# openhumanoids/pronto

Hardware: AMD Instinct MI355X
Metric: EKF predict+update steps/sec (batched filters), 15-state, 1000 Hz IMU (higher is better)
Workload: dtype f64

## Files before the change

pronto_amd/csrc/rbis_coop.hpp:

```cpp
#pragma once

#include "rbis_device.hpp"

namespace pb {

template <int NS>
struct Coop {
  static constexpr bool HB = (NS == 21);
  static constexpr int NSC = HB ? 15 : 9;
  static constexpr int NPC = NSC * (NSC + 1) / 2;
  static constexpr int NB_ = HB ? 6 : 0;
  static constexpr bool LL_IN_P = !HB;
  static constexpr int XCH_LLI = 9 + 3 * NSC;
  static constexpr int NXCH = 9 + 3 * NSC + (LL_IN_P ? 1 : 0);
  PB_HD static constexpr int fullc(int s) { return core_full(s); }
  PB_HD static constexpr int fullp(int p) { return passive_full(p); }
};

struct ProcBlocks {
  double a_mw[3];
  double a_g[3];
  double a_mv[3];
  double A_R[9];
  double A_RV[9];
// ... 73 lines not shown
using CorrGpfYawPos = Corr<false, 5, 6, 7, 8>;
using CorrGpfChiPos = Corr<false, 3, 4, 5, 6, 7, 8>;
using CorrGpfZ = Corr<false, 8>;
struct CorrInputs {
  double z[6], rd[6], qm[4];
  double ro[15] = { 0, 0, 0, 0, 0, 0, 0, 0, 0, 0, 0, 0, 0, 0, 0 };
  bool upd;
};
template <int NS, class CORR>
struct CoopX {
  using C = Coop<NS>;
  static constexpr int M = CORR::M;
  static constexpr int X2_L = C::NXCH, X2_ID = X2_L + M * (M - 1) / 2, X2_YD = X2_ID + M, X2_W = X2_YD + M,
                       X2_LLI = X2_W + C::NSC * M;
  static constexpr int NXCH = (M == 0) ? C::NXCH : X2_LLI + (C::LL_IN_P ? 1 : 0);
  static constexpr int XCH_LEG = C::NXCH, XCH_FOOT = XCH_LEG + 10, NXCH_LEG = (NXCH > XCH_FOOT + 14) ? NXCH : XCH_FOOT + 14;
  static constexpr int X6_ID = 0, X6_YD = 3, X6_LLI = 6, X6_A = 9;
};

#if defined(__HIP_DEVICE_COMPILE__)
__device__ __forceinline__ void pb_pin(double &v) { asm volatile("" : "+v"(v)); }
#else
inline void pb_pin(double &) {}
#endif
struct NoPredStore {
  static constexpr bool on = false;
  PB_HD void operator()(int, double) const {}
};
struct SixIn {
  double z[3] = { 0.0, 0.0, 0.0 }, r = 1.0;
  bool on = false;
};

template <int NS, bool UPDATE, class CORR = NoCorr, bool PREDICT = true, bool LEG = false, int SIX = 0, class LD, class ST, class XW, class XR, class SYNC,
          class SP = NoPredStore>
PB_HD void coop_role_core(LD ld, ST st, XW xw, XR xr, SYNC sync, const StepInputs &in, const Consts &k,
                          const CorrInputs &cin_ = CorrInputs(), SP sp = SP())
{
  static_assert(!SP::on || (PREDICT && UPDATE && !LEG && SIX == 0), "the predicted rows: the fused step, with or without a CORR stage");
  static_assert(!LEG || (UPDATE && PREDICT), "the odometry wave feeds a predict + update step");
  static_assert(SIX == 0 || (UPDATE && PREDICT), "the six-row leg-odometry modes ride on a predict + velocity update");
  static_assert(SIX != 2 || (CORR::M == 3 && !CORR::ORIENT), "SIX == 2: the second block is a 3-row vector block of role C's states");
  static_assert(SIX != 1 || CORR::M == 0, "SIX == 1 has no CORR stage");
  using L = Lay<NS>;
  using C = Coop<NS>;
  constexpr int NSC = C::NSC;
  static_assert(PREDICT || !UPDATE, "the leg-odometry update rides behind a predict");
  static_assert(PREDICT || CORR::M > 0, "nothing to do");
  double x[NS], q[4], ll = 0.0;
#pragma unroll
  for (int i = 0; i < NS; i++) x[i] = ld(L::OFF_VEC + i);
#pragma unroll
  for (int i = 0; i < 4; i++) q[i] = ld(L::OFF_QUAT + i);
  if constexpr (!C::LL_IN_P) ll = ld(L::OFF_LL);
  double Pc[C::NPC];
#pragma unroll
  for (int i = 0; i < NSC; i++)
#pragma unroll
    for (int j = 0; j <= i; j++) Pc[pk(i, j)] = ld(L::OFF_P + pk(C::fullc(i), C::fullc(j)));

  if constexpr (PREDICT) {
  ProcBlocks f;
  make_proc_blocks<NS>(x, q, in.dt, k, f);
  {
    const int src[2] = { 0, 1 };
    const int kind[2] = { 0, 0 };
    double A[2][9];
#pragma unroll
// ... 20 lines not shown
#pragma unroll
    for (int i = 0; i < 9; i++) { A[0][i] = f.a_mw[i % 3]; A[1][i] = f.a_g[i % 3]; }
    RowOp<NSC, 0, 2>::apply(Pc, src, kind, A);
    const int src2[1] = { 1 };
    const int kind2[1] = { 1 };
    double A2[1][9];
#pragma unroll
    for (int i = 0; i < 9; i++) A2[0][i] = f.a_mw[i % 3];
    RowOp<NSC, 1, 1>::apply(Pc, src2, kind2, A2);
  }
  {
    const double qgd = in.qg * in.dt, qad = in.qa * in.dt;
    const double vv = f.v[0] * f.v[0] + f.v[1] * f.v[1] + f.v[2] * f.v[2];
#pragma unroll
    for (int r = 0; r < 3; r++)
#pragma unroll
      for (int c = 0; c <= r; c++) Pc[pk(r, c)] += qgd * ((r == c ? vv : 0.0) - f.v[r] * f.v[c]) + (r == c ? qad : 0.0);
    const double m[9] = { 0, f.v[2], -f.v[1], -f.v[2], 0, f.v[0], f.v[1], -f.v[0], 0 };
#pragma unroll
    for (int r = 0; r < 3; r++)
#pragma unroll
      for (int c = 0; c < 3; c++)
        if (r != c) Pc[pk(3 + r, c)] += qgd * m[3 * r + c];
#pragma unroll
    for (int r = 0; r < 3; r++) Pc[pk(3 + r, 3 + r)] += qgd;
    if constexpr (C::HB) {
#pragma unroll
      for (int r = 0; r < 3; r++) {
        Pc[pk(9 + r, 9 + r)] += in.qbg * in.dt;
        Pc[pk(12 + r, 12 + r)] += in.qba * in.dt;
      }
    }
  }
  ins_update_state<NS>(x, q, in.gyro, in.accel, in.dt, k);
  }
  if constexpr (SP::on) {
#pragma unroll
    for (int i = 0; i < NSC; i++)
#pragma unroll
      for (int j = 0; j <= i; j++) sp(L::OFF_P + pk(C::fullc(i), C::fullc(j)), Pc[pk(i, j)]);
#pragma unroll
    for (int i = 0; i < NSC; i++) sp(L::OFF_VEC + C::fullc(i), x[C::fullc(i)]);
#pragma unroll
    for (int i = 0; i < 4; i++) sp(L::OFF_QUAT + i, q[i]);
    if constexpr (!C::LL_IN_P) sp(L::OFF_LL, ll);
  }

  double dfull[NS];
#pragma unroll
  for (int i = 0; i < NS; i++) dfull[i] = 0.0;
  bool upd1 = false;
  double leg2[5] = { 0.0, 0.0, 0.0, 1.0, 0.0 };
  if constexpr (UPDATE) {
    double resid[3], S[6], d[3], y[3], id[3], yd[3];
    double mz[3], mr[3];
    double dx1[SIX == 1 ? NSC : 1], idw = 0.0;
    dx1[0] = 0.0;
    bool mupd = in.upd;
    if constexpr (LEG || SIX == 1) {
#pragma unroll
      for (int i = 0; i < C::NPC; i++) pb_pin(Pc[i]);
#pragma unroll
      for (int i = 0; i < 9; i++) pb_pin(x[C::fullc(i)]);
#pragma unroll
      for (int i = 0; i < 4; i++) pb_pin(q[i]);
      sync();
    }
// ... 21 lines not shown
    }
    if constexpr (LEG) {
      const double r = xr(CoopX<NS, CORR>::XCH_LEG + 3);
      mupd = in.upd && xr(CoopX<NS, CORR>::XCH_LEG + 4) != 0.0;
      if constexpr (SIX == 2) {
#pragma unroll
        for (int i = 0; i < 5; i++) leg2[i] = xr(CoopX<NS, CORR>::XCH_LEG + 5 + i);
      }
#pragma unroll
      for (int i = 0; i < 3; i++) { mz[i] = xr(CoopX<NS, CORR>::XCH_LEG + i); mr[i] = r; }
    } else {
#pragma unroll
      for (int i = 0; i < 3; i++) { mz[i] = in.z[i]; mr[i] = in.rd[i]; }
    }
#pragma unroll
    for (int i = 0; i < 3; i++) resid[i] = mupd ? mz[i] - (SIX == 1 ? x[3 + i] + dx1[i] : x[3 + i]) : 0.0;
#pragma unroll
    for (int i = 0; i < 3; i++)
#pragma unroll
      for (int j = 0; j <= i; j++) S[pk(i, j)] = Pc[pk(i, j)] + (i == j ? (mupd ? mr[i] : 1.0) : 0.0);
    ldlt<3>(S, d);
    double quad = 0.0, det = 1.0;
#pragma unroll
    for (int kk = 0; kk < 3; kk++) {
      double s = resid[kk];
#pragma unroll
      for (int j = 0; j < kk; j++) s -= S[pk(kk, j)] * y[j];
      y[kk] = mupd ? s : 0.0;
      id[kk] = mupd ? 1.0 / d[kk] : 0.0;
      yd[kk] = y[kk] * id[kk];
      det *= d[kk];
      quad += s * s * id[kk];
    }
    const double lli = -log(det) - quad;
    if constexpr (C::LL_IN_P) xw(C::XCH_LLI, lli);
    else if (mupd) ll += lli;
    double W[NSC][3];
#pragma unroll
    for (int i = 0; i < NSC; i++)
#pragma unroll
      for (int kk = 0; kk < 3; kk++) {
        double s = Pc[pk(i, kk)];
#pragma unroll
        for (int j = 0; j < kk; j++) s -= W[i][j] * S[pk(kk, j)];
        W[i][kk] = s;
      }
    xw(0, S[pk(1, 0)]); xw(1, S[pk(2, 0)]); xw(2, S[pk(2, 1)]);
#pragma unroll
    for (int kk = 0; kk < 3; kk++) { xw(3 + kk, id[kk]); xw(6 + kk, yd[kk]); }
#pragma unroll
    for (int i = 0; i < NSC; i++)
#pragma unroll
      for (int kk = 0; kk < 3; kk++) xw(9 + 3 * i + kk, W[i][kk]);
    sync();
#pragma unroll
    for (int i = 0; i < NSC; i++) {
      double wd[3];
#pragma unroll
      for (int kk = 0; kk < 3; kk++) wd[kk] = W[i][kk] * id[kk];
      dfull[C::fullc(i)] = fma(W[i][2], yd[2], fma(W[i][1], yd[1], W[i][0] * yd[0])) + (SIX == 1 ? dx1[i] : 0.0);
#pragma unroll
      for (int j = 0; j <= i; j++) {
        double acc = Pc[pk(i, j)];
#pragma unroll
        for (int kk = 0; kk < 3; kk++) acc = fma(-wd[kk], W[j][kk], acc);
        if constexpr (CORR::M == 0) st(L::OFF_P + pk(C::fullc(i), C::fullc(j)), acc);
        else Pc[pk(i, j)] = acc;
      }
    }
    upd1 = mupd || idw != 0.0;
    if constexpr (SIX != 2) {
      if (upd1) add_delta<NS>(x, q, dfull, k.chi_tol);
    }
  }
  if constexpr (CORR::M > 0) {
    constexpr int M = CORR::M;
    using CX = CoopX<NS, CORR>;
    CorrInputs cin = cin_;
    if constexpr (LEG && SIX == 2) {
#pragma unroll
      for (int i = 0; i < 3; i++) { cin.z[i] = leg2[i]; cin.rd[i] = leg2[3]; }
      cin.upd = in.upd && leg2[4] != 0.0;
    }
    double r2[M], S2[M * (M + 1) / 2], d2[M], y2[M], id2[M], yd2[M];
    double dq3[3] = { 0.0, 0.0, 0.0 };
    if constexpr (CORR::ORIENT) subtract_quats(cin.qm, q, dq3);
#pragma unroll
    for (int kk = 0; kk < M; kk++) {
      const int ii = C::fullc(CORR::sub[kk]);
      const double r = (CORR::ORIENT && ii >= 6 && ii <= 8) ? dq3[ii - 6] : cin.z[kk] - (SIX == 2 ? x[ii] + dfull[ii] : x[ii]);
      r2[kk] = cin.upd ? r : 0.0;
    }
#pragma unroll
    for (int i = 0; i < M; i++)
#pragma unroll
      for (int j = 0; j <= i; j++)
        S2[pk(i, j)] = Pc[pk(CORR::sub[i], CORR::sub[j])] + (i == j ? (cin.upd ? cin.rd[i] : 1.0) : (cin.upd ? cin.ro[i * (i - 1) / 2 + j] : 0.0));
    ldlt<M>(S2, d2);
    double quad2 = 0.0, det2 = 1.0;
#pragma unroll
    for (int kk = 0; kk < M; kk++) {
      double s2 = r2[kk];
#pragma unroll
      for (int j = 0; j < kk; j++) s2 -= S2[pk(kk, j)] * y2[j];
      y2[kk] = cin.upd ? s2 : 0.0;
// ... 40 lines not shown
      for (int kk = 0; kk < M; kk++) wd2[kk] = (W2_LDS ? xr(CX::X2_W + M * i + kk) : W2[i][kk]) * id2[kk];
#pragma unroll
      for (int j = 0; j <= i; j++) {
        double acc = Pc[pk(i, j)];
#pragma unroll
        for (int kk = 0; kk < M; kk++) acc = fma(-wd2[kk], W2_LDS ? xr(CX::X2_W + M * j + kk) : W2[j][kk], acc);
        st(L::OFF_P + pk(C::fullc(i), C::fullc(j)), acc);
      }
    }
    if constexpr (SIX == 2) {
#pragma unroll
      for (int i = 0; i < NS; i++) dfull2[i] += dfull[i];
      if (upd1 || cin.upd) add_delta<NS>(x, q, dfull2, k.chi_tol);
    } else {
      if (cin.upd) add_delta<NS>(x, q, dfull2, k.chi_tol);
    }
  }
  if constexpr (!UPDATE && CORR::M == 0) {
#pragma unroll
    for (int i = 0; i < NSC; i++)
#pragma unroll
      for (int j = 0; j <= i; j++) st(L::OFF_P + pk(C::fullc(i), C::fullc(j)), Pc[pk(i, j)]);
    sync();
  }
#pragma unroll
  for (int i = 0; i < 9; i++) st(L::OFF_VEC + C::fullc(i), x[C::fullc(i)]);
#pragma unroll
  for (int i = 0; i < 4; i++) st(L::OFF_QUAT + i, q[i]);
  if constexpr (!C::LL_IN_P) st(L::OFF_LL, ll);
#pragma unroll
  for (int i = 9; i < NSC; i++) st(L::OFF_VEC + C::fullc(i), x[C::fullc(i)]);
}

template <int NS, bool UPDATE, class CORR = NoCorr, bool PREDICT = true, int SIX = 0, class LD, class ST, class XW, class XR, class SYNC,
          class SP = NoPredStore>
PB_HD void coop_role_passive_x(LD ld, ST st, XW xw, XR xr, SYNC sync, const StepInputs &in, const Consts &k,
                               const CorrInputs &cin = CorrInputs(), const SixIn &six = SixIn(), SP sp = SP())
{
  static_assert(!SP::on || (PREDICT && UPDATE && SIX == 0), "the predicted rows: the fused step, with or without a CORR stage");
  static_assert(SIX != 1 || (UPDATE && PREDICT && CORR::M == 0), "SIX == 1 rides on a predict + velocity update");
  using L = Lay<NS>;
  using C = Coop<NS>;
  double x[NS], q[4] = { 1.0, 0.0, 0.0, 0.0 };
#pragma unroll
  for (int i = 0; i < NS; i++) x[i] = 0.0;
  if constexpr (PREDICT) {
#pragma unroll
    for (int i = 0; i < NS; i++) x[i] = ld(L::OFF_VEC + i);
#pragma unroll
    for (int i = 0; i < 4; i++) q[i] = ld(L::OFF_QUAT + i);
  } else {
#pragma unroll
    for (int i = 0; i < 6; i++) x[C::fullp(i)] = ld(L::OFF_VEC + C::fullp(i));
  }
  constexpr int NSB = C::HB ? 5 : 3;
  double X[NSB][2][9];
#pragma unroll
  for (int sb = 0; sb < NSB; sb++)
#pragma unroll
    for (int J = 0; J < 2; J++)
#pragma unroll
      for (int r = 0; r < 3; r++)
#pragma unroll
        for (int c = 0; c < 3; c++) X[sb][J][3 * r + c] = ld(L::OFF_P + pk(C::fullc(3 * sb + r), C::fullp(3 * J + c)));
  double Ppp[21];
#pragma unroll
  for (int i = 0; i < 6; i++)
#pragma unroll
    for (int j = 0; j <= i; j++) Ppp[pk(i, j)] = ld(L::OFF_P + pk(C::fullp(i), C::fullp(j)));
  double ll = 0.0;
  if constexpr (C::LL_IN_P) ll = ld(L::OFF_LL);

  double xp[6];
  if constexpr (!PREDICT) {
#pragma unroll
    for (int i = 0; i < 6; i++) xp[i] = x[C::fullp(i)];
  }
  if constexpr (PREDICT) {
  ProcBlocks f;
  make_proc_blocks<NS>(x, q, in.dt, k, f);
#pragma unroll
  for (int J = 0; J < 2; J++) {
    double nD[9], nV[9], nC[9];
#pragma unroll
    for (int i = 0; i < 9; i++) { nD[i] = X[2][J][i]; nV[i] = X[0][J][i]; nC[i] = X[1][J][i]; }
    mat_mul_acc(f.A_R, X[0][J], nD);
    mat_mul_acc(f.A_RV, X[1][J], nD);
    hat_mul_acc(f.a_mw, X[0][J], nV);
    hat_mul_acc(f.a_g, X[1][J], nV);
    hat_mul_acc(f.a_mw, X[1][J], nC);
    if constexpr (C::HB) {
      hat_mul_acc(f.a_mv, X[3][J], nV);
#pragma unroll
      for (int i = 0; i < 9; i++) {
        nV[i] -= in.dt * X[4][J][i];
        nC[i] -= in.dt * X[3][J][i];
      }
    }
#pragma unroll
    for (int i = 0; i < 9; i++) { X[2][J][i] = nD[i]; X[0][J][i] = nV[i]; X[1][J][i] = nC[i]; }
  }
#pragma unroll
  for (int r = 0; r < 3; r++)
#pragma unroll
    for (int c = 0; c <= r; c++) {
      Ppp[pk(r, c)] = (r == c) ? in.qg : 0.0;
      Ppp[pk(3 + r, 3 + c)] = (r == c) ? in.qa : 0.0;
    }
#pragma unroll
  for (int i = 0; i < 3; i++) {
    xp[i] = in.gyro[i] - (C::HB ? x[15 + i] : 0.0);
    xp[3 + i] = in.accel[i] - (C::HB ? x[18 + i] : 0.0);
  }
  }
  if constexpr (SP::on) {
#pragma unroll
    for (int J = 0; J < 2; J++)
#pragma unroll
      for (int sb = 0; sb < NSB; sb++)
#pragma unroll
        for (int r = 0; r < 3; r++)
#pragma unroll
          for (int c = 0; c < 3; c++) sp(L::OFF_P + pk(C::fullc(3 * sb + r), C::fullp(3 * J + c)), X[sb][J][3 * r + c]);
#pragma unroll
    for (int i = 0; i < 6; i++)
#pragma unroll
      for (int j = 0; j <= i; j++) sp(L::OFF_P + pk(C::fullp(i), C::fullp(j)), Ppp[pk(i, j)]);
    if constexpr (C::LL_IN_P) sp(L::OFF_LL, ll);
#pragma unroll
    for (int i = 0; i < 6; i++) sp(L::OFF_VEC + C::fullp(i), xp[i]);
  }

  if constexpr (SIX == 1) {
    using CX = CoopX<NS, CORR>;
    const double idw = six.on ? 1.0 / (in.qg + six.r) : 0.0;
    double ydw[3], quad = 0.0;
#pragma unroll
    for (int kk = 0; kk < 3; kk++) {
      const double res = six.on ? six.z[kk] - xp[kk] : 0.0;
      ydw[kk] = res * idw;
      quad = fma(res, ydw[kk], quad);
    }
    const double dw = in.qg + six.r;
    const double lliw = six.on ? -log(dw * dw * dw) - quad : 0.0;
    xw(CX::X6_ID, idw);
// ... 9 lines not shown
        for (int kk = 0; kk < 3; kk++) xw(CX::X6_A + 3 * (3 * sb + r) + kk, X[sb][0][3 * r + kk]);
    sync();
    const double keep = fma(-in.qg, idw, 1.0);
#pragma unroll
    for (int sb = 0; sb < NSB; sb++)
#pragma unroll
      for (int r = 0; r < 3; r++) {
        const double ad[3] = { X[sb][0][3 * r] * idw, X[sb][0][3 * r + 1] * idw, X[sb][0][3 * r + 2] * idw };
#pragma unroll
        for (int c = 0; c < 3; c++) {
          X[sb][1][3 * r + c] = fma(-ad[2], Ppp[pk(3 + c, 2)], fma(-ad[1], Ppp[pk(3 + c, 1)], fma(-ad[0], Ppp[pk(3 + c, 0)], X[sb][1][3 * r + c])));
          X[sb][0][3 * r + c] *= keep;
        }
      }
#pragma unroll
    for (int r = 0; r < 3; r++) {
      const double ad[3] = { Ppp[pk(3 + r, 0)] * idw, Ppp[pk(3 + r, 1)] * idw, Ppp[pk(3 + r, 2)] * idw };
      xp[3 + r] += fma(Ppp[pk(3 + r, 2)], ydw[2], fma(Ppp[pk(3 + r, 1)], ydw[1], Ppp[pk(3 + r, 0)] * ydw[0]));
#pragma unroll
      for (int c = 0; c <= r; c++)
        Ppp[pk(3 + r, 3 + c)] = fma(-ad[2], Ppp[pk(3 + c, 2)], fma(-ad[1], Ppp[pk(3 + c, 1)], fma(-ad[0], Ppp[pk(3 + c, 0)], Ppp[pk(3 + r, 3 + c)])));
    }
#pragma unroll
    for (int r = 0; r < 3; r++) {
#pragma unroll
      for (int c = 0; c < 3; c++) Ppp[pk(3 + r, c)] *= keep;
      Ppp[pk(r, r)] = in.qg * keep;
      xp[r] = fma(in.qg, ydw[r], xp[r]);
    }
  }
  if constexpr (!UPDATE && CORR::M == 0) sync();
  if constexpr (UPDATE) {
    sync();
    const double L10 = xr(0), L20 = xr(1), L21 = xr(2);
    double id[3], yd[3];
#pragma unroll
    for (int kk = 0; kk < 3; kk++) { id[kk] = xr(3 + kk); yd[kk] = xr(6 + kk); }
    double Wp[6][3];
#pragma unroll
    for (int pi = 0; pi < 6; pi++) {
      const double c0 = X[0][pi / 3][0 * 3 + pi % 3], c1 = X[0][pi / 3][1 * 3 + pi % 3], c2 = X[0][pi / 3][2 * 3 + pi % 3];
      Wp[pi][0] = c0;
      Wp[pi][1] = c1 - Wp[pi][0] * L10;
      Wp[pi][2] = c2 - Wp[pi][0] * L20 - Wp[pi][1] * L21;
      xp[pi] += fma(Wp[pi][2], yd[2], fma(Wp[pi][1], yd[1], Wp[pi][0] * yd[0]));
    }
    if constexpr (C::LL_IN_P) {
      const double lli = xr(C::XCH_LLI);
      if (in.upd) ll += lli;
    }
#pragma unroll
    for (int J = 0; J < 2; J++)
#pragma unroll
      for (int sb = 0; sb < NSB; sb++)
#pragma unroll
        for (int r = 0; r < 3; r++) {
          double wd[3];
#pragma unroll
          for (int kk = 0; kk < 3; kk++) wd[kk] = xr(9 + 3 * (3 * sb + r) + kk) * id[kk];
#pragma unroll
          for (int c = 0; c < 3; c++) {
            double acc = X[sb][J][3 * r + c];
#pragma unroll
            for (int kk = 0; kk < 3; kk++) acc = fma(-wd[kk], Wp[3 * J + c][kk], acc);
            if constexpr (CORR::M == 0) st(L::OFF_P + pk(C::fullc(3 * sb + r), C::fullp(3 * J + c)), acc);
            else X[sb][J][3 * r + c] = acc;
          }
        }
#pragma unroll
    for (int i = 0; i < 6; i++) {
      double wd[3];
#pragma unroll
      for (int kk = 0; kk < 3; kk++) wd[kk] = Wp[i][kk] * id[kk];
#pragma unroll
      for (int j = 0; j <= i; j++) {
        double acc = Ppp[pk(i, j)];
#pragma unroll
        for (int kk = 0; kk < 3; kk++) acc = fma(-wd[kk], Wp[j][kk], acc);
        if constexpr (CORR::M == 0) st(L::OFF_P + pk(C::fullp(i), C::fullp(j)), acc);
        else Ppp[pk(i, j)] = acc;
      }
    }
  }
  if constexpr (CORR::M > 0) {
    constexpr int M = CORR::M;
    using CX = CoopX<NS, CORR>;
    sync();
    double id2[M], yd2[M], L2[M * (M - 1) / 2 + 1];
#pragma unroll
    for (int i = 0; i < M * (M - 1) / 2; i++) L2[i] = xr(CX::X2_L + i);
#pragma unroll
    for (int kk = 0; kk < M; kk++) { id2[kk] = xr(CX::X2_ID + kk); yd2[kk] = xr(CX::X2_YD + kk); }
    if constexpr (C::LL_IN_P) {
      const double lli2 = xr(CX::X2_LLI);
      if (cin.upd) ll += lli2;
    }
    double W2p[6][M];
#pragma unroll
    for (int pi = 0; pi < 6; pi++) {
      double dxs = 0.0;
#pragma unroll
// ... 29 lines not shown
#pragma unroll
      for (int kk = 0; kk < M; kk++) wd2[kk] = W2p[i][kk] * id2[kk];
#pragma unroll
      for (int j = 0; j <= i; j++) {
        double acc = Ppp[pk(i, j)];
#pragma unroll
        for (int kk = 0; kk < M; kk++) acc = fma(-wd2[kk], W2p[j][kk], acc);
        st(L::OFF_P + pk(C::fullp(i), C::fullp(j)), acc);
      }
    }
  }
  if constexpr (!UPDATE && CORR::M == 0) {
#pragma unroll
    for (int J = 0; J < 2; J++)
#pragma unroll
      for (int sb = 0; sb < NSB; sb++)
#pragma unroll
        for (int r = 0; r < 3; r++)
#pragma unroll
          for (int c = 0; c < 3; c++) st(L::OFF_P + pk(C::fullc(3 * sb + r), C::fullp(3 * J + c)), X[sb][J][3 * r + c]);
#pragma unroll
    for (int i = 0; i < 6; i++)
#pragma unroll
      for (int j = 0; j <= i; j++) st(L::OFF_P + pk(C::fullp(i), C::fullp(j)), Ppp[pk(i, j)]);
  }
  if constexpr (C::LL_IN_P) st(L::OFF_LL, ll);
#pragma unroll
  for (int i = 0; i < 6; i++) st(L::OFF_VEC + C::fullp(i), xp[i]);
}
template <int NS, bool UPDATE, class CORR = NoCorr, bool PREDICT = true, class LD, class ST, class XR, class SYNC, class SP = NoPredStore>
PB_HD void coop_role_passive(LD ld, ST st, XR xr, SYNC sync, const StepInputs &in, const Consts &k,
                             const CorrInputs &cin = CorrInputs(), SP sp = SP())
{
  coop_role_passive_x<NS, UPDATE, CORR, PREDICT, 0>(ld, st, [](int, double) {}, xr, sync, in, k, cin, SixIn(), sp);
}

}
```

pronto_amd/csrc/rbis_device.hpp:

```cpp
#pragma once

#include <cmath>
#include <type_traits>
#include <utility>

#if defined(__HIPCC__)
#include <hip/hip_runtime.h>
#define PB_HD __host__ __device__ __forceinline__
#else
#define PB_HD inline
#endif

namespace pb {

template <int NS>
struct Lay {
  static constexpr int NB = NS / 3;
  static constexpr int NP = NS * (NS + 1) / 2;
  static constexpr int OFF_VEC = 0;
  static constexpr int OFF_QUAT = NS;
  static constexpr int OFF_LL = NS + 4;
  static constexpr int OFF_P = NS + 5;
  static constexpr int NC = NS + 5 + NP;
};
// ... 109 lines not shown
};

enum { BW = 0, BV = 1, BCHI = 2, BPOS = 3, BACC = 4, BBG = 5, BBA = 6 };

struct Consts {
  double g;
  double chi_tol;
  const double *qblk = nullptr;
  int xcd_remap = 0;
  int half_tiles = 0;
};

PB_HD void quat_mul(const double (&a)[4], const double (&b)[4], double (&o)[4])
{
  const double w = a[0] * b[0] - a[1] * b[1] - a[2] * b[2] - a[3] * b[3];
  const double x = a[0] * b[1] + a[1] * b[0] + a[2] * b[3] - a[3] * b[2];
  const double y = a[0] * b[2] + a[2] * b[0] + a[3] * b[1] - a[1] * b[3];
  const double z = a[0] * b[3] + a[3] * b[0] + a[1] * b[2] - a[2] * b[1];
  o[0] = w; o[1] = x; o[2] = y; o[3] = z;
}

PB_HD void quat_to_rot(const double (&q)[4], double (&R)[9])
{
  const double w = q[0], x = q[1], y = q[2], z = q[3];
  const double tx = 2 * x, ty = 2 * y, tz = 2 * z;
  const double twx = tx * w, twy = ty * w, twz = tz * w;
  const double txx = tx * x, txy = ty * x, txz = tz * x;
  const double tyy = ty * y, tyz = tz * y, tzz = tz * z;
  R[0] = 1 - (tyy + tzz); R[1] = txy - twz;       R[2] = txz + twy;
  R[3] = txy + twz;       R[4] = 1 - (txx + tzz); R[5] = tyz - twx;
  R[6] = txz - twy;       R[7] = tyz + twx;       R[8] = 1 - (txx + tyy);
}

PB_HD void sincos_joint(double x, double &s, double &c)
{
  const double kf = rint(x * 6.36619772367581382433e-01);
  double r = fma(-kf, 1.57079632673412561417e+00, x);
  r = fma(-kf, 6.07710050650619224932e-11, r);
  const double z = r * r;
  double ps = 1.58969099521155010221e-10;
  ps = fma(ps, z, -2.50507602534068634195e-08);
  ps = fma(ps, z, 2.75573137070700676789e-06);
  ps = fma(ps, z, -1.98412698298579493134e-04);
  ps = fma(ps, z, 8.33333333332248946124e-03);
  ps = fma(ps, z, -1.66666666666666324348e-01);
  const double sn = fma(r * z, ps, r);
  double pc = -1.13596475577881948265e-11;
  pc = fma(pc, z, 2.08757232129817482790e-09);
  pc = fma(pc, z, -2.75573143513906633035e-07);
  pc = fma(pc, z, 2.48015872894767294178e-05);
  pc = fma(pc, z, -1.38888888888741095749e-03);
  pc = fma(pc, z, 4.16666666666666019037e-02);
  const double cs = fma(z * z, pc, fma(-0.5, z, 1.0));
  const int k = (int) kf & 3;
  const double a = (k & 1) ? cs : sn, b = (k & 1) ? sn : cs;
  s = (k & 2) ? -a : a;
  c = ((k + 1) & 2) ? -b : b;
}

PB_HD void fold_chi(double (&chi)[3], double (&q)[4], double tol)
{
  const double n = sqrt(chi[0] * chi[0] + chi[1] * chi[1] + chi[2] * chi[2]);
  if (n > tol) {
    double s, c;
    sincos_joint(0.5 * n, s, c);
    const double f = s / n;
    const double dq[4] = { c, f * chi[0], f * chi[1], f * chi[2] };
    double o[4];
    quat_mul(q, dq, o);
    q[0] = o[0]; q[1] = o[1]; q[2] = o[2]; q[3] = o[3];
    chi[0] = chi[1] = chi[2] = 0.0;
  }
}

template <int NS>
PB_HD void add_delta(double (&x)[NS], double (&q)[4], double (&d)[NS], double tol)
{
  double dchi[3] = { d[6], d[7], d[8] };
  double dq[4] = { 1.0, 0.0, 0.0, 0.0 };
  fold_chi(dchi, dq, tol);
  d[6] = dchi[0]; d[7] = dchi[1]; d[8] = dchi[2];
#pragma unroll
  for (int i = 0; i < NS; i++) x[i] += d[i];
  double chi[3] = { x[6], x[7], x[8] };
  fold_chi(chi, q, tol);
  x[6] = chi[0]; x[7] = chi[1]; x[8] = chi[2];
  double o[4];
  quat_mul(q, dq, o);
  q[0] = o[0]; q[1] = o[1]; q[2] = o[2]; q[3] = o[3];
}

PB_HD void subtract_quats(const double (&q1)[4], const double (&q2)[4], double (&out)[3])
{
  const double n2 = q2[0] * q2[0] + q2[1] * q2[1] + q2[2] * q2[2] + q2[3] * q2[3];
  const double in2 = 1.0 / n2;
  const double q2i[4] = { q2[0] * in2, -q2[1] * in2, -q2[2] * in2, -q2[3] * in2 };
  double r[4];
  quat_mul(q2i, q1, r);
  const double n = sqrt(r[1] * r[1] + r[2] * r[2] + r[3] * r[3]);
  if (n != 0.0) {
    double angle = 2.0 * atan2(n, fabs(r[0]));
    if (angle >= 3.141592653589793) angle -= 6.283185307179586;
    const double f = (r[0] < 0 ? -angle : angle) / n;
    out[0] = r[1] * f; out[1] = r[2] * f; out[2] = r[3] * f;
  } else {
    out[0] = out[1] = out[2] = 0.0;
  }
}


template <int NS>
PB_HD void ins_update_state(double (&x)[NS], double (&q)[4], const double (&gyro)[3], const double (&accel)[3],
                            double dt, const Consts &k)
{
  double R[9];
  quat_to_rot(q, R);
  double w[3], a[3];
#pragma unroll
  for (int i = 0; i < 3; i++) {
    w[i] = gyro[i] - (NS == 21 ? x[15 + i] : 0.0);
    a[i] = accel[i] - (NS == 21 ? x[18 + i] : 0.0);
  }
  const double v[3] = { x[3], x[4], x[5] };
  const double wxv[3] = { w[1] * v[2] - w[2] * v[1], w[2] * v[0] - w[0] * v[2], w[0] * v[1] - w[1] * v[0] };
  double d[NS];
#pragma unroll
  for (int i = 0; i < NS; i++) d[i] = 0.0;
#pragma unroll
  for (int i = 0; i < 3; i++) {
    d[3 + i] = ((-wxv[i]) + ((-k.g) * R[6 + i] + a[i])) * dt;
    d[6 + i] = w[i] * dt;
    d[9 + i] = (R[3 * i] * v[0] + R[3 * i + 1] * v[1] + R[3 * i + 2] * v[2]) * dt;
    x[i] = w[i];
    x[12 + i] = a[i];
  }
  add_delta<NS>(x, q, d, k.chi_tol);
}

template <int NS>
PB_HD void ins_update_quat(const double (&chi_prior)[3], const double (&gyro_bias)[3], double (&q)[4], const double (&gyro)[3], double dt,
                           const Consts &k)
{
  double dchi[3], chi[3];
#pragma unroll
  for (int i = 0; i < 3; i++) dchi[i] = (gyro[i] - (NS == 21 ? gyro_bias[i] : 0.0)) * dt;
  double dq[4] = { 1.0, 0.0, 0.0, 0.0 };
  fold_chi(dchi, dq, k.chi_tol);
#pragma unroll
  for (int i = 0; i < 3; i++) chi[i] = chi_prior[i] + dchi[i];
  fold_chi(chi, q, k.chi_tol);
  double o[4];
  quat_mul(q, dq, o);
  q[0] = o[0]; q[1] = o[1]; q[2] = o[2]; q[3] = o[3];
}

template <int NS, int I, int NSRC>
struct RowOp {
  static constexpr int NB = NS / 3;
  static constexpr int NP = NS * (NS + 1) / 2;

  PB_HD static bool nz(int kind, int r, int c) { return kind == 0 || (kind == 1 && r != c) || (kind == 2 && r == c); }

  PB_HD static double el(const double (&A)[9], int kind, int r, int c)
  {
    if (kind == 0) return A[3 * r + c];
    if (kind == 2) return A[0];
    if (r == 0 && c == 1) return -A[2];
    if (r == 0 && c == 2) return A[1];
    if (r == 1 && c == 0) return A[2];
// ... 291 lines not shown
```

pronto_amd/csrc/rbis_replay_kernels.hpp:

```cpp
#pragma once

#include "rbis_tile_io.hpp"
#include "rbis_coop.hpp"
#include "rbis_quad.hpp"

namespace pb {

template <int NS>
__global__ __launch_bounds__(64, 1) void k_replay_fused(double *__restrict__ st, int B, int T,
                                                        const double *__restrict__ imu, const double *__restrict__ lo,
                                                        const uint8_t *__restrict__ mask, double qg, double qa, double qbg,
                                                        double qba, Consts k)
{
  using L = Lay<NS>;
  const unsigned b = blockIdx.x * blockDim.x + threadIdx.x;
  if (b >= (unsigned) B) return;
  const unsigned bo = b * 8u, B8 = (unsigned) B * 8u;
  TileIO<NS, 0, 0> io(st, st, blockIdx.x, threadIdx.x);
  io.template need<0, Slots<NS>::NROW>();
  double x[NS], q[4], ll, P[L::NP];
#pragma unroll
  for (int i = 0; i < NS; i++) x[i] = io.ld(L::OFF_VEC + i);
#pragma unroll
  for (int i = 0; i < 4; i++) q[i] = io.ld(L::OFF_QUAT + i);
// ... 9 lines not shown
  auto fetch = [&](int t, double (&dst)[13], bool &u) {
    const rsrc_t ri = mkbuf(imu + (size_t) t * 7 * B, 7u * B8);
    const rsrc_t rl = mkbuf(lo + (size_t) t * 6 * B, 6u * B8);
#pragma unroll
    for (int i = 0; i < 7; i++) dst[i] = ldg(ri, i * B8, bo);
#pragma unroll
    for (int i = 0; i < 6; i++) dst[7 + i] = ldg(rl, i * B8, bo);
    u = (mask == nullptr) || (mask[(size_t) t * B + b] != 0);
  };
  fetch(0, in, upd);
  for (int t = 0; t < T; t++) {
    if (t > 0) fetch(t, in, upd);
    const double gyro[3] = { in[0], in[1], in[2] }, accel[3] = { in[3], in[4], in[5] };
    imu_process_step<NS>(x, q, P, gyro, accel, in[6], qg, qa, qbg, qba, k);
    double resid[3], S[6];
#pragma unroll
    for (int i = 0; i < 3; i++) resid[i] = upd ? in[7 + i] - x[3 + i] : 0.0;
#pragma unroll
    for (int i = 0; i < 3; i++)
#pragma unroll
      for (int j = 0; j <= i; j++) S[pk(i, j)] = P[pk(3 + i, 3 + j)] + (i == j ? (upd ? in[10 + i] : 1.0) : 0.0);
    measurement_update<NS, 3>(x, q, P, ll, resid, S, IdxVel{}, k, NoSink(), upd);
  }
#pragma unroll
  for (int i = 0; i < L::NP; i++) io.st(L::OFF_P + i, P[i]);
#pragma unroll
  for (int i = 0; i < NS; i++) io.st(L::OFF_VEC + i, x[i]);
#pragma unroll
  for (int i = 0; i < 4; i++) io.st(L::OFF_QUAT + i, q[i]);
  io.st(L::OFF_LL, ll);
}

template <int NS>
__global__ __launch_bounds__(128, 1) void k_replay_coop(double *st, int B, int T, const double *__restrict__ imu,
                                                        const double *__restrict__ lo, const uint8_t *__restrict__ mask,
                                                        double qg, double qa, double qbg, double qba, Consts k, SlotOut so)
{
  using L = Lay<NS>;
  using C = Coop<NS>;
  using SL = Slots<NS>;
  __shared__ double xch[C::NXCH][64];
  __shared__ double xst[NS + 4][64];
  const int role = __builtin_amdgcn_readfirstlane((int) (threadIdx.x >> 6));
  const unsigned lane = threadIdx.x & 63u;
  const unsigned tile = blockIdx.x;
  const unsigned b = tile * 64u + lane;
  const unsigned bo = b * 8u, B8 = (unsigned) B * 8u;
  TileIO<NS, 0, 0, true> io(st, st, tile, lane);
  double q4[4] = { qg, qa, qbg, qba };
  if (k.qblk != nullptr) {
    const rsrc_t rq = mkbuf(k.qblk, 4u * B8);
#pragma unroll
    for (int i = 0; i < 4; i++) q4[i] = ldg(rq, (unsigned) i * B8, bo);
  }
  auto sync = []() { __syncthreads(); };
  auto xw = [lane](int s, double v) { xch[s][lane] = v; };
  auto xrd = [lane](int s) { return xch[s][lane]; };
  auto inputs = [&](int t) {
    const rsrc_t ri = mkbuf(imu + (size_t) t * 7 * B, 7u * B8);
    const rsrc_t rl = mkbuf(lo + (size_t) t * 6 * B, 6u * B8);
    StepInputs in;
#pragma unroll
    for (int i = 0; i < 3; i++) {
      in.gyro[i] = ldg(ri, i * B8, bo);
      in.accel[i] = ldg(ri, (3 + i) * B8, bo);
      in.z[i] = ldg(rl, i * B8, bo);
      in.rd[i] = ldg(rl, (3 + i) * B8, bo);
    }
    in.dt = ldg(ri, 6u * B8, bo);
    in.upd = (b < (unsigned) B) && (mask == nullptr || mask[(size_t) t * B + b] != 0);
    in.qg = q4[0]; in.qa = q4[1]; in.qbg = q4[2]; in.qba = q4[3];
    return in;
  };
  if (role == 0) {
    double V[L::NC];
    io.template need<0, SL::ROW_SPLIT>();
    static_for<SL::NSLOT>([&](auto I) {
      constexpr int slot = decltype(I)::value, comp = SL::T.comp_of[slot];
      if constexpr (comp >= 0 && SL::T.role2[slot] == 0) V[comp] = io.ld(comp);
    });
    auto ld = [&V](int comp) { return V[comp]; };
    auto stf = [&V](int comp, double v) { V[comp] = v; };
    for (int t = 0; t < T; t++) {
      const StepInputs in = inputs(t);
#pragma unroll
      for (int i = 0; i < C::NSC; i++) xst[C::fullc(i)][lane] = V[L::OFF_VEC + C::fullc(i)];
#pragma unroll
      for (int i = 0; i < 4; i++) xst[NS + i][lane] = V[L::OFF_QUAT + i];
      __syncthreads();
#pragma unroll
      for (int i = 0; i < 6; i++) V[L::OFF_VEC + C::fullp(i)] = xst[C::fullp(i)][lane];
      coop_role_core<NS, true>(ld, stf, xw, xrd, sync, in, k);
      if (so.base != nullptr) {
        TileIO<NS, 0, MemHint<MH_STREAM_NT>::SA, true> ios(st, so.base + (size_t) t * so.stride, tile, lane);
        static_for<SL::NSLOT>([&](auto I) {
          constexpr int slot = decltype(I)::value, comp = SL::T.comp_of[slot];
          if constexpr (comp >= 0 && SL::T.role2[slot] == 0) ios.st(comp, V[comp]);
        });
      }
    }
    static_for<SL::NSLOT>([&](auto I) {
      constexpr int slot = decltype(I)::value, comp = SL::T.comp_of[slot];
      if constexpr (comp >= 0 && SL::T.role2[slot] == 0) io.st(comp, V[comp]);
    });
  } else {
    double V[L::NC];
    io.template need<SL::ROW_SPLIT, SL::NROW>();
    static_for<SL::NSLOT>([&](auto I) {
      constexpr int slot = decltype(I)::value, comp = SL::T.comp_of[slot];
      if constexpr (comp >= 0 && SL::T.role2[slot] == 1) V[comp] = io.ld(comp);
    });
    auto ld = [&V](int comp) { return V[comp]; };
    auto stf = [&V](int comp, double v) { V[comp] = v; };
    for (int t = 0; t < T; t++) {
      const StepInputs in = inputs(t);
#pragma unroll
      for (int i = 0; i < 6; i++) xst[C::fullp(i)][lane] = V[L::OFF_VEC + C::fullp(i)];
      __syncthreads();
#pragma unroll
      for (int i = 0; i < C::NSC; i++) V[L::OFF_VEC + C::fullc(i)] = xst[C::fullc(i)][lane];
#pragma unroll
      for (int i = 0; i < 4; i++) V[L::OFF_QUAT + i] = xst[NS + i][lane];
      coop_role_passive<NS, true>(ld, stf, xrd, sync, in, k);
      if (so.base != nullptr) {
        TileIO<NS, 0, MemHint<MH_STREAM_NT>::SA, true> ios(st, so.base + (size_t) t * so.stride, tile, lane);
        static_for<SL::NSLOT>([&](auto I) {
          constexpr int slot = decltype(I)::value, comp = SL::T.comp_of[slot];
          if constexpr (comp >= 0 && SL::T.role2[slot] == 1) ios.st(comp, V[comp]);
        });
      }
    }
    static_for<SL::NSLOT>([&](auto I) {
      constexpr int slot = decltype(I)::value, comp = SL::T.comp_of[slot];
      if constexpr (comp >= 0 && SL::T.role2[slot] == 1) io.st(comp, V[comp]);
    });
  }
}

template <int OCC>
__global__ __launch_bounds__(256, OCC) void k_replay_quad(double *st, int B, int T, const double *__restrict__ imu,
                                                        const double *__restrict__ lo, const uint8_t *__restrict__ mask,
                                                        double qg, double qa, double qbg, double qba, Consts k, SlotOut so)
{
  constexpr int NS = 21;
  using L = Lay<NS>;
  using SL = Slots<NS>;
  __shared__ double xch[Quad::NXCH][64];
  __shared__ double xst[NS + 4][64];
  const int role = __builtin_amdgcn_readfirstlane((int) (threadIdx.x >> 6));
  const unsigned lane = threadIdx.x & 63u;
  const unsigned tile = blockIdx.x;
  const unsigned b = tile * 64u + lane;
  const unsigned bo = b * 8u, B8 = (unsigned) B * 8u;
  TileIO<NS, 0, 0> io(st, st, tile, lane);
  double q4[4] = { qg, qa, qbg, qba };
  if (k.qblk != nullptr) {
// ... 76 lines not shown
```

Measured before the change: 2.726 billion.

## Restructure 15-state coop replay for two blocks per CU with prefetch and deferred passive work

```diff
diff --git a/pronto_amd/csrc/rbis_coop.hpp b/pronto_amd/csrc/rbis_coop.hpp
--- a/pronto_amd/csrc/rbis_coop.hpp
+++ b/pronto_amd/csrc/rbis_coop.hpp
@@ -129,8 +129,8 @@
   bool on = false;
 };
 
-template <int NS, bool UPDATE, class CORR = NoCorr, bool PREDICT = true, bool LEG = false, int SIX = 0, class LD, class ST, class XW, class XR, class SYNC,
-          class SP = NoPredStore>
+template <int NS, bool UPDATE, class CORR = NoCorr, bool PREDICT = true, bool LEG = false, int SIX = 0, bool SEQ = false, class LD, class ST, class XW, class XR,
+          class SYNC, class SP = NoPredStore>
 PB_HD void coop_role_core(LD ld, ST st, XW xw, XR xr, SYNC sync, const StepInputs &in, const Consts &k,
                           const CorrInputs &cin_ = CorrInputs(), SP sp = SP())
 {
@@ -217,7 +217,23 @@
       }
     }
   }
-  ins_update_state<NS>(x, q, in.gyro, in.accel, in.dt, k);
+  if constexpr (SEQ) {
+#pragma unroll
+    for (int i = 0; i < C::NPC; i++) pb_pin(Pc[i]);
+#pragma unroll
+    for (int i = 0; i < 9; i++) pb_pin(x[C::fullc(i)]);
+#pragma unroll
+    for (int i = 0; i < 4; i++) pb_pin(q[i]);
+  }
+  ins_update_state<NS, SEQ>(x, q, in.gyro, in.accel, in.dt, k);
+  if constexpr (SEQ) {
+#pragma unroll
+    for (int i = 0; i < 9; i++) pb_pin(x[C::fullc(i)]);
+#pragma unroll
+    for (int i = 0; i < 4; i++) pb_pin(q[i]);
+#pragma unroll
+    for (int i = 0; i < C::NPC; i++) pb_pin(Pc[i]);
+  }
   }
   if constexpr (SP::on) {
 #pragma unroll
@@ -305,9 +321,14 @@
       det *= d[kk];
       quad += s * s * id[kk];
     }
+    if constexpr (SEQ && C::LL_IN_P) {
+      xw(C::XCH_LLI, det);
+      xw(C::NXCH, quad);
+    } else {
     const double lli = -log(det) - quad;
     if constexpr (C::LL_IN_P) xw(C::XCH_LLI, lli);
     else if (mupd) ll += lli;
+    }
     double W[NSC][3];
 #pragma unroll
     for (int i = 0; i < NSC; i++)
@@ -342,8 +363,14 @@
       }
     }
     upd1 = mupd || idw != 0.0;
+    if constexpr (SEQ) {
+#pragma unroll
+      for (int i = 0; i < 9; i++) { pb_pin(x[C::fullc(i)]); pb_pin(dfull[C::fullc(i)]); }
+#pragma unroll
+      for (int i = 0; i < 4; i++) pb_pin(q[i]);
+    }
     if constexpr (SIX != 2) {
-      if (upd1) add_delta<NS>(x, q, dfull, k.chi_tol);
+      if (upd1) add_delta<NS, SEQ>(x, q, dfull, k.chi_tol);
     }
   }
   if constexpr (CORR::M > 0) {
@@ -450,13 +477,14 @@
   for (int i = 9; i < NSC; i++) st(L::OFF_VEC + C::fullc(i), x[C::fullc(i)]);
 }
 
-template <int NS, bool UPDATE, class CORR = NoCorr, bool PREDICT = true, int SIX = 0, class LD, class ST, class XW, class XR, class SYNC,
-          class SP = NoPredStore>
+template <int NS, bool UPDATE, class CORR = NoCorr, bool PREDICT = true, int SIX = 0, bool SEQ = false, class LD, class ST, class XW, class XR,
+          class SYNC, class SP = NoPredStore>
 PB_HD void coop_role_passive_x(LD ld, ST st, XW xw, XR xr, SYNC sync, const StepInputs &in, const Consts &k,
                                const CorrInputs &cin = CorrInputs(), const SixIn &six = SixIn(), SP sp = SP())
 {
   static_assert(!SP::on || (PREDICT && UPDATE && SIX == 0), "the predicted rows: the fused step, with or without a CORR stage");
   static_assert(SIX != 1 || (UPDATE && PREDICT && CORR::M == 0), "SIX == 1 rides on a predict + velocity update");
+  static_assert(!SEQ || (UPDATE && PREDICT && CORR::M == 0 && SIX == 0 && !SP::on && Coop<NS>::LL_IN_P), "SEQ: the plain fused step");
   using L = Lay<NS>;
   using C = Coop<NS>;
   double x[NS], q[4] = { 1.0, 0.0, 0.0, 0.0 };
@@ -482,12 +510,14 @@
 #pragma unroll
         for (int c = 0; c < 3; c++) X[sb][J][3 * r + c] = ld(L::OFF_P + pk(C::fullc(3 * sb + r), C::fullp(3 * J + c)));
   double Ppp[21];
+  if constexpr (!SEQ) {
 #pragma unroll
   for (int i = 0; i < 6; i++)
 #pragma unroll
     for (int j = 0; j <= i; j++) Ppp[pk(i, j)] = ld(L::OFF_P + pk(C::fullp(i), C::fullp(j)));
+  }
   double ll = 0.0;
-  if constexpr (C::LL_IN_P) ll = ld(L::OFF_LL);
+  if constexpr (C::LL_IN_P && !SEQ) ll = ld(L::OFF_LL);
 
   double xp[6];
   if constexpr (!PREDICT) {
@@ -518,6 +548,7 @@
 #pragma unroll
     for (int i = 0; i < 9; i++) { X[2][J][i] = nD[i]; X[0][J][i] = nV[i]; X[1][J][i] = nC[i]; }
   }
+  if constexpr (!SEQ) {
 #pragma unroll
   for (int r = 0; r < 3; r++)
 #pragma unroll
@@ -529,6 +560,7 @@
   for (int i = 0; i < 3; i++) {
     xp[i] = in.gyro[i] - (C::HB ? x[15 + i] : 0.0);
     xp[3 + i] = in.accel[i] - (C::HB ? x[18 + i] : 0.0);
+  }
   }
   }
   if constexpr (SP::on) {
@@ -604,6 +636,21 @@
   if constexpr (!UPDATE && CORR::M == 0) sync();
   if constexpr (UPDATE) {
     sync();
+    if constexpr (SEQ) {
+#pragma unroll
+      for (int r = 0; r < 3; r++)
+#pragma unroll
+        for (int c = 0; c <= r; c++) {
+          Ppp[pk(r, c)] = (r == c) ? in.qg : 0.0;
+          Ppp[pk(3 + r, 3 + c)] = (r == c) ? in.qa : 0.0;
+        }
+#pragma unroll
+      for (int i = 0; i < 3; i++) {
+        xp[i] = in.gyro[i];
+        xp[3 + i] = in.accel[i];
+      }
+      ll = ld(L::OFF_LL);
+    }
     const double L10 = xr(0), L20 = xr(1), L21 = xr(2);
     double id[3], yd[3];
 #pragma unroll
@@ -618,7 +665,7 @@
       xp[pi] += fma(Wp[pi][2], yd[2], fma(Wp[pi][1], yd[1], Wp[pi][0] * yd[0]));
     }
     if constexpr (C::LL_IN_P) {
-      const double lli = xr(C::XCH_LLI);
+      const double lli = SEQ ? -log_khere(xr(C::XCH_LLI)) - xr(C::NXCH) : xr(C::XCH_LLI);
       if (in.upd) ll += lli;
     }
 #pragma unroll
@@ -639,6 +686,12 @@
             else X[sb][J][3 * r + c] = acc;
           }
         }
+    if constexpr (SEQ) {
+#pragma unroll
+      for (int r = 0; r < 3; r++)
+#pragma unroll
+        for (int c = 0; c < 3; c++) Ppp[pk(3 + r, c)] = ld(L::OFF_P + pk(C::fullp(3 + r), C::fullp(c)));
+    }
 #pragma unroll
     for (int i = 0; i < 6; i++) {
       double wd[3];
@@ -734,7 +787,7 @@
 PB_HD void coop_role_passive(LD ld, ST st, XR xr, SYNC sync, const StepInputs &in, const Consts &k,
                              const CorrInputs &cin = CorrInputs(), SP sp = SP())
 {
-  coop_role_passive_x<NS, UPDATE, CORR, PREDICT, 0>(ld, st, [](int, double) {}, xr, sync, in, k, cin, SixIn(), sp);
+  coop_role_passive_x<NS, UPDATE, CORR, PREDICT, 0, false>(ld, st, [](int, double) {}, xr, sync, in, k, cin, SixIn(), sp);
 }
 
 }
diff --git a/pronto_amd/csrc/rbis_device.hpp b/pronto_amd/csrc/rbis_device.hpp
--- a/pronto_amd/csrc/rbis_device.hpp
+++ b/pronto_amd/csrc/rbis_device.hpp
@@ -165,25 +165,76 @@
   R[6] = txz - twy;       R[7] = tyz + twx;       R[8] = 1 - (txx + tyy);
 }
 
+template <bool KHERE>
+struct KHere {
+  unsigned zero = 0;
+  PB_HD KHere()
+  {
+#if defined(__HIP_DEVICE_COMPILE__)
+    if constexpr (KHERE) asm volatile("" : "+s"(zero));
+#endif
+  }
+  PB_HD double operator()(double v) const
+  {
+    if constexpr (KHERE) {
+      const unsigned long long u = __builtin_bit_cast(unsigned long long, v);
+      const unsigned lo = (unsigned) u ^ zero, hi = (unsigned) (u >> 32) ^ zero;
+      return __builtin_bit_cast(double, ((unsigned long long) hi << 32) | lo);
+    } else {
+      return v;
+    }
+  }
+};
+
+PB_HD double log_khere(double x)
+{
+  const KHere<true> K;
+  int e;
+  double m = frexp(x, &e);
+  const bool lowhalf = m < K(7.07106781186547572737e-01);
+  m = lowhalf ? m + m : m;
+  const double dk = (double) (lowhalf ? e - 1 : e);
+  const double f = m - 1.0;
+  const double s = f / (2.0 + f);
+  const double z = s * s, w = z * z;
+  double t1 = K(1.531383769920937332e-01);
+  t1 = fma(w, t1, K(2.222219843214978396e-01));
+  t1 = fma(w, t1, K(3.999999999940941908e-01));
+  t1 = w * t1;
+  double t2 = K(1.479819860511658591e-01);
+  t2 = fma(w, t2, K(1.818357216161805012e-01));
+  t2 = fma(w, t2, K(2.857142874366239149e-01));
+  t2 = fma(w, t2, K(6.666666666666735130e-01));
+  t2 = z * t2;
+  const double R = t2 + t1;
+  const double hfsq = 0.5 * f * f;
+  const double r = dk * K(6.93147180369123816490e-01) - ((hfsq - (s * (hfsq + R) + dk * K(1.90821492927058770002e-10))) - f);
+  const double inf = K(__builtin_huge_val());
+  const double edge = (x == 0.0) ? -inf : (x == inf ? inf : K(__builtin_nan("")));
+  return (x > 0.0 && x < inf) ? r : edge;
+}
+
+template <bool KHERE = false>
 PB_HD void sincos_joint(double x, double &s, double &c)
 {
-  const double kf = rint(x * 6.36619772367581382433e-01);
-  double r = fma(-kf, 1.57079632673412561417e+00, x);
-  r = fma(-kf, 6.07710050650619224932e-11, r);
+  const KHere<KHERE> K;
+  const double kf = rint(x * K(6.36619772367581382433e-01));
+  double r = fma(-kf, K(1.57079632673412561417e+00), x);
+  r = fma(-kf, K(6.07710050650619224932e-11), r);
   const double z = r * r;
-  double ps = 1.58969099521155010221e-10;
-  ps = fma(ps, z, -2.50507602534068634195e-08);
-  ps = fma(ps, z, 2.75573137070700676789e-06);
-  ps = fma(ps, z, -1.98412698298579493134e-04);
-  ps = fma(ps, z, 8.33333333332248946124e-03);
-  ps = fma(ps, z, -1.66666666666666324348e-01);
+  double ps = K(1.58969099521155010221e-10);
+  ps = fma(ps, z, K(-2.50507602534068634195e-08));
+  ps = fma(ps, z, K(2.75573137070700676789e-06));
+  ps = fma(ps, z, K(-1.98412698298579493134e-04));
+  ps = fma(ps, z, K(8.33333333332248946124e-03));
+  ps = fma(ps, z, K(-1.66666666666666324348e-01));
   const double sn = fma(r * z, ps, r);
-  double pc = -1.13596475577881948265e-11;
-  pc = fma(pc, z, 2.08757232129817482790e-09);
-  pc = fma(pc, z, -2.75573143513906633035e-07);
-  pc = fma(pc, z, 2.48015872894767294178e-05);
-  pc = fma(pc, z, -1.38888888888741095749e-03);
-  pc = fma(pc, z, 4.16666666666666019037e-02);
+  double pc = K(-1.13596475577881948265e-11);
+  pc = fma(pc, z, K(2.08757232129817482790e-09));
+  pc = fma(pc, z, K(-2.75573143513906633035e-07));
+  pc = fma(pc, z, K(2.48015872894767294178e-05));
+  pc = fma(pc, z, K(-1.38888888888741095749e-03));
+  pc = fma(pc, z, K(4.16666666666666019037e-02));
   const double cs = fma(z * z, pc, fma(-0.5, z, 1.0));
   const int k = (int) kf & 3;
   const double a = (k & 1) ? cs : sn, b = (k & 1) ? sn : cs;
@@ -191,12 +242,13 @@
   c = ((k + 1) & 2) ? -b : b;
 }
 
+template <bool KHERE = false>
 PB_HD void fold_chi(double (&chi)[3], double (&q)[4], double tol)
 {
   const double n = sqrt(chi[0] * chi[0] + chi[1] * chi[1] + chi[2] * chi[2]);
   if (n > tol) {
     double s, c;
-    sincos_joint(0.5 * n, s, c);
+    sincos_joint<KHERE>(0.5 * n, s, c);
     const double f = s / n;
     const double dq[4] = { c, f * chi[0], f * chi[1], f * chi[2] };
     double o[4];
@@ -206,17 +258,17 @@
   }
 }
 
-template <int NS>
+template <int NS, bool KHERE = false>
 PB_HD void add_delta(double (&x)[NS], double (&q)[4], double (&d)[NS], double tol)
 {
   double dchi[3] = { d[6], d[7], d[8] };
   double dq[4] = { 1.0, 0.0, 0.0, 0.0 };
-  fold_chi(dchi, dq, tol);
+  fold_chi<KHERE>(dchi, dq, tol);
   d[6] = dchi[0]; d[7] = dchi[1]; d[8] = dchi[2];
 #pragma unroll
   for (int i = 0; i < NS; i++) x[i] += d[i];
   double chi[3] = { x[6], x[7], x[8] };
-  fold_chi(chi, q, tol);
+  fold_chi<KHERE>(chi, q, tol);
   x[6] = chi[0]; x[7] = chi[1]; x[8] = chi[2];
   double o[4];
   quat_mul(q, dq, o);
@@ -242,7 +294,7 @@
 }
 
 
-template <int NS>
+template <int NS, bool KHERE = false>
 PB_HD void ins_update_state(double (&x)[NS], double (&q)[4], const double (&gyro)[3], const double (&accel)[3],
                             double dt, const Consts &k)
 {
@@ -267,7 +319,7 @@
     x[i] = w[i];
     x[12 + i] = a[i];
   }
-  add_delta<NS>(x, q, d, k.chi_tol);
+  add_delta<NS, KHERE>(x, q, d, k.chi_tol);
 }
 
 template <int NS>
diff --git a/pronto_amd/csrc/rbis_replay_kernels.hpp b/pronto_amd/csrc/rbis_replay_kernels.hpp
--- a/pronto_amd/csrc/rbis_replay_kernels.hpp
+++ b/pronto_amd/csrc/rbis_replay_kernels.hpp
@@ -65,31 +65,32 @@
 }
 
 template <int NS>
-__global__ __launch_bounds__(128, 1) void k_replay_coop(double *st, int B, int T, const double *__restrict__ imu,
-                                                        const double *__restrict__ lo, const uint8_t *__restrict__ mask,
-                                                        double qg, double qa, double qbg, double qba, Consts k, SlotOut so)
+__global__ __launch_bounds__(128, NS == 15 ? 2 : 1) void k_replay_coop(double *st, int B, int T, const double *__restrict__ imu,
+                                                                       const double *__restrict__ lo, const uint8_t *__restrict__ mask,
+                                                                       double qg, double qa, double qbg, double qba, Consts k, SlotOut so)
 {
   using L = Lay<NS>;
   using C = Coop<NS>;
   using SL = Slots<NS>;
-  __shared__ double xch[C::NXCH][64];
+  constexpr bool TWO = (NS == 15);
+  __shared__ double xch[C::NXCH + (TWO ? 1 : 0)][64];
   __shared__ double xst[NS + 4][64];
+  __shared__ double xpp[TWO ? 10 : 1][64];
   const int role = __builtin_amdgcn_readfirstlane((int) (threadIdx.x >> 6));
   const unsigned lane = threadIdx.x & 63u;
-  const unsigned tile = blockIdx.x;
+  const unsigned tile = TWO ? xcd_workgroup(k) : blockIdx.x;
   const unsigned b = tile * 64u + lane;
   const unsigned bo = b * 8u, B8 = (unsigned) B * 8u;
   TileIO<NS, 0, 0, true> io(st, st, tile, lane);
   double q4[4] = { qg, qa, qbg, qba };
-  if (k.qblk != nullptr) {
+  if (!TWO && k.qblk != nullptr) {
     const rsrc_t rq = mkbuf(k.qblk, 4u * B8);
 #pragma unroll
     for (int i = 0; i < 4; i++) q4[i] = ldg(rq, (unsigned) i * B8, bo);
   }
-  auto sync = []() { __syncthreads(); };
   auto xw = [lane](int s, double v) { xch[s][lane] = v; };
   auto xrd = [lane](int s) { return xch[s][lane]; };
-  auto inputs = [&](int t) {
+  auto inputs = [&](int t, bool meas) {
     const rsrc_t ri = mkbuf(imu + (size_t) t * 7 * B, 7u * B8);
     const rsrc_t rl = mkbuf(lo + (size_t) t * 6 * B, 6u * B8);
     StepInputs in;
@@ -97,12 +98,22 @@
     for (int i = 0; i < 3; i++) {
       in.gyro[i] = ldg(ri, i * B8, bo);
       in.accel[i] = ldg(ri, (3 + i) * B8, bo);
-      in.z[i] = ldg(rl, i * B8, bo);
-      in.rd[i] = ldg(rl, (3 + i) * B8, bo);
+      in.z[i] = meas ? ldg(rl, i * B8, bo) : 0.0;
+      in.rd[i] = meas ? ldg(rl, (3 + i) * B8, bo) : 1.0;
     }
     in.dt = ldg(ri, 6u * B8, bo);
-    in.upd = (b < (unsigned) B) && (mask == nullptr || mask[(size_t) t * B + b] != 0);
-    in.qg = q4[0]; in.qa = q4[1]; in.qbg = q4[2]; in.qba = q4[3];
+    if constexpr (TWO) {
+      in.upd = (b < (unsigned) B) &&
+               (mask == nullptr || __builtin_amdgcn_raw_buffer_load_b8(mkbuf(mask + (size_t) t * B, (unsigned) B), b, 0, 0) != 0);
+      in.qg = qg; in.qa = qa; in.qbg = qbg; in.qba = qba;
+      if (k.qblk != nullptr) {
+        const rsrc_t rq = mkbuf(k.qblk, 4u * B8);
+        in.qg = ldg(rq, 0u, bo); in.qa = ldg(rq, B8, bo);
+      }
+    } else {
+      in.upd = (b < (unsigned) B) && (mask == nullptr || mask[(size_t) t * B + b] != 0);
+      in.qg = q4[0]; in.qa = q4[1]; in.qbg = q4[2]; in.qba = q4[3];
+    }
     return in;
   };
   if (role == 0) {
@@ -113,9 +124,15 @@
       if constexpr (comp >= 0 && SL::T.role2[slot] == 0) V[comp] = io.ld(comp);
     });
     auto ld = [&V](int comp) { return V[comp]; };
-    auto stf = [&V](int comp, double v) { V[comp] = v; };
+    auto stf = [&V](int comp, double v) { if (TWO) pb_pin(v); V[comp] = v; };
+    StepInputs nxt;
+    if (TWO) nxt = inputs(0, true);
     for (int t = 0; t < T; t++) {
-      const StepInputs in = inputs(t);
+      const StepInputs in = TWO ? nxt : inputs(t, true);
+      auto sync = [&]() {
+        __syncthreads();
+        if (TWO && t + 1 < T) nxt = inputs(t + 1, true);
+      };
 #pragma unroll
       for (int i = 0; i < C::NSC; i++) xst[C::fullc(i)][lane] = V[L::OFF_VEC + C::fullc(i)];
 #pragma unroll
@@ -123,7 +140,7 @@
       __syncthreads();
 #pragma unroll
       for (int i = 0; i < 6; i++) V[L::OFF_VEC + C::fullp(i)] = xst[C::fullp(i)][lane];
-      coop_role_core<NS, true>(ld, stf, xw, xrd, sync, in, k);
+      coop_role_core<NS, true, NoCorr, true, false, 0, TWO>(ld, stf, xw, xrd, sync, in, k);
       if (so.base != nullptr) {
         TileIO<NS, 0, MemHint<MH_STREAM_NT>::SA, true> ios(st, so.base + (size_t) t * so.stride, tile, lane);
         static_for<SL::NSLOT>([&](auto I) {
@@ -143,10 +160,34 @@
       constexpr int slot = decltype(I)::value, comp = SL::T.comp_of[slot];
       if constexpr (comp >= 0 && SL::T.role2[slot] == 1) V[comp] = io.ld(comp);
     });
-    auto ld = [&V](int comp) { return V[comp]; };
-    auto stf = [&V](int comp, double v) { V[comp] = v; };
+    auto park = [](int comp) {
+      int f = (TWO && comp == L::OFF_LL) ? 9 : -1;
+      for (int r = 0; r < 3; r++)
+        for (int c = 0; c < 3; c++)
+          if (TWO && comp == L::OFF_P + pk(C::fullp(3 + r), C::fullp(c))) f = 3 * r + c;
+      return f;
+    };
+    auto ld = [&V, &park, lane](int comp) { return park(comp) >= 0 ? xpp[park(comp)][lane] : V[comp]; };
+    auto stf = [&V, &park, lane](int comp, double v) {
+      V[comp] = v;
+      if (park(comp) >= 0) xpp[park(comp)][lane] = v;
+    };
+    static_for<L::NC>([&](auto I) {
+      constexpr int comp = decltype(I)::value;
+      if (park(comp) >= 0) xpp[park(comp)][lane] = V[comp];
+    });
     for (int t = 0; t < T; t++) {
-      const StepInputs in = inputs(t);
+      StepInputs in;
+      if constexpr (TWO) {
+        in.dt = ldg(mkbuf(imu + (size_t) t * 7 * B, 7u * B8), 6u * B8, bo);
+        in.upd = false;
+      } else {
+        in = inputs(t, false);
+      }
+      auto sync = [&]() {
+        if constexpr (TWO) in = inputs(t, false);
+        __syncthreads();
+      };
 #pragma unroll
       for (int i = 0; i < 6; i++) xst[C::fullp(i)][lane] = V[L::OFF_VEC + C::fullp(i)];
       __syncthreads();
@@ -154,7 +195,7 @@
       for (int i = 0; i < C::NSC; i++) V[L::OFF_VEC + C::fullc(i)] = xst[C::fullc(i)][lane];
 #pragma unroll
       for (int i = 0; i < 4; i++) V[L::OFF_QUAT + i] = xst[NS + i][lane];
-      coop_role_passive<NS, true>(ld, stf, xrd, sync, in, k);
+      coop_role_passive_x<NS, true, NoCorr, true, 0, TWO>(ld, stf, [](int, double) {}, xrd, sync, in, k);
       if (so.base != nullptr) {
         TileIO<NS, 0, MemHint<MH_STREAM_NT>::SA, true> ios(st, so.base + (size_t) t * so.stride, tile, lane);
         static_for<SL::NSLOT>([&](auto I) {
```

New measurement: 2.734 billion (median of 4 runs). No clear change (+0.3%).
